# nh273/caro-ai

Hardware: AMD Instinct MI355X
Metric: self-play MCTS node-expansions/sec/GPU (Connect4, 200 sims/move); 1->8 GPU scaling (higher is better)
Workload: dtype f32

## Files before the change

caro_ai_amd/csrc/caro_engine.hip:

```cpp
#include <hip/hip_runtime.h>

#include <cstddef>
#include <cstdio>
#include <cstdlib>
#include <cstring>
#include <string>
#include <type_traits>
#include <vector>

#include "../../include/caro_hip.h"
#include "../../include/caro_noise.h"
#include "caro_rules.h"
#include "caro_variants.h"

namespace caro {

constexpr uint32_t NSTRONG = 1u << 30;
constexpr uint32_t NMASK = NSTRONG - 1u;
constexpr int ST_DROPPED = 0, ST_TERMINAL = 1, ST_LEAF = 2;
constexpr int MAXB = 64;
constexpr int DONE_HELD = 3;

enum Counter { C_SIMS, C_LEVELS, C_EXPANSIONS, C_TERMINALS, C_DROPPED, C_OVERFLOW, C_PLIES, C_FINISHED, C_N };

// ... 1099 lines not shown
    float* dst = planes + (size_t)rowi * 2 * HW;
    for (int i = tid; i < 2 * HW; i += blockDim.x) dst[i] = R::plane(v.gp, brd, who, i / HW, i % HW);
    if (leaf_keys && tid < KW) leaf_keys[(size_t)rowi * KW + tid] = v.d_key[di * KW + tid];
  }
}

template <int AP>
__device__ __forceinline__ void backup_path(const View& v, int t, float value, bool strong_val, const int32_t* pn,
                                            const int32_t* pa, int len) {
  float cur = -value;
  for (int i = len - 1; i >= 0; --i) {
    uint32_t* row = v.edges + (ebase(v, t) + pn[i]) * 4 * AP;
    const int a = pa[i];
    const uint32_t nraw = row[4 * a];
    const int n = (int)(nraw & NMASK) + 1;
    const uint32_t strong = (nraw & NSTRONG) | (strong_val ? NSTRONG : 0u);
    const float w = __uint_as_float(row[4 * a + 1]) + cur;
    const float q = w / (float)n;
    row[4 * a] = (uint32_t)n | strong;
    row[4 * a + 1] = __float_as_uint(w);
    row[4 * a + 2] = __float_as_uint(q);
    cur = -cur;
  }
}
template <int AP>
__device__ __forceinline__ void backup_path_rec(const View& v, int t, float value, bool strong_val, const uint4* rec,
                                                int len) {
  float cur = -value;
  for (int i = len - 1; i >= 0; --i) {
    const uint32_t na = rec[i].x;
    uint32_t* row = v.edges + (ebase(v, t) + (na & 0xFFFFFFu)) * 4 * AP;
    const int a = (int)(na >> 24);
    const uint32_t nraw = row[4 * a];
    const int n = (int)(nraw & NMASK) + 1;
    const uint32_t strong = (nraw & NSTRONG) | (strong_val ? NSTRONG : 0u);
    const float w = __uint_as_float(row[4 * a + 1]) + cur;
    row[4 * a] = (uint32_t)n | strong;
    row[4 * a + 1] = __float_as_uint(w);
    row[4 * a + 2] = __float_as_uint(w / (float)n);
    cur = -cur;
  }
}

template <class GEO>
struct ExpandPre {
  static constexpr int NPR = (MAXB * 0 + 64 * GEO::APL + 63) / 64;
  uint4 rec;
  typename GEO::R::Board brd;
  float row_val;
  uint4 p0, p1;
  float pr[NPR];
  int nleaf;
};
template <class GEO, bool ONE>
__device__ __forceinline__ ExpandPre<GEO> expand_preload(const View& v, int g, int B, int off, const float* __restrict__ probs,
                                                         const float* __restrict__ values) {
  using R = typename GEO::R;
  constexpr int KW = GEO::KW, AP = GEO::AP;
  ExpandPre<GEO> e;
  const int lane = threadIdx.x;
  e.nleaf = v.g_nleaf[g];
  e.rec = make_uint4(ST_DROPPED, 0u, 0u, 0u);
  e.row_val = 0.f;
#pragma unroll
  for (int w = 0; w < KW; ++w) e.brd.w[w] = 0;
  if (lane < B) {
    const size_t di = (size_t)g * v.maxB + lane;
    e.rec = v.d_rec[di];
    e.brd = load_board<R>(v.d_key + di * KW);
    if ((long long)off + lane < (long long)v.G * v.maxB) e.row_val = values[off + lane];
  }
  e.p0 = e.p1 = make_uint4(0u, 0u, 0u, 0u);
  if (B <= 8 && lane < 64 && (lane >> 3) < B) {
    const uint4* pr = v.path_rec + ((size_t)g * v.maxB + (lane >> 3)) * v.maxd;
    if ((lane & 7) < v.maxd) e.p0 = pr[lane & 7];
    if (8 + (lane & 7) < v.maxd) e.p1 = pr[8 + (lane & 7)];
  }
#pragma unroll
  for (int k = 0; k < ExpandPre<GEO>::NPR; ++k) {
    e.pr[k] = 0.f;
    if (ONE) {
      const int idx = lane + 64 * k, b = idx / AP, a = idx - b * AP;
      if (idx < B * AP && a < v.A && lane < 64) e.pr[k] = probs[(size_t)(off + b) * v.A + a];
    }
  }
  return e;
}

template <class GEO, bool ONE = false, class OPT = TreeFull>
__device__ __forceinline__ void expand_body(const View& v, GameRegs<GEO>& gr, int B, const ExpandPre<GEO>& pre, int off,
                                            const float* __restrict__ probs) {
  using R = typename GEO::R;
  using Board = typename R::Board;
  constexpr int AP = GEO::AP, KW = GEO::KW;
  constexpr int MAXE = GEO::APL > 1 ? 256 : 512;
  constexpr int MAXB = geo_max_batch<GEO>();
  __shared__ int e_node[MAXE];
  __shared__ short e_act[MAXE];
  __shared__ float e_val[MAXE];
  __shared__ unsigned char e_strong[MAXE];
  __shared__ uint32_t e_n[MAXE], e_w[MAXE];
  __shared__ int s_total;
  __shared__ uint64_t s_brd[MAXB][KW];
  __shared__ int s_node[MAXB], s_row[MAXB];
  __shared__ uint32_t s_home[MAXB];
  __shared__ unsigned char s_free[MAXB];
  __shared__ int q_len[MAXB], q_off[MAXB], q_b[MAXB];
  __shared__ float q_val[MAXB];
  __shared__ unsigned char q_strong[MAXB];
  __shared__ int s_nq;
  __shared__ uint4 s_p0[64], s_p1[64];
  __shared__ float s_rowval[MAXB];
  const int g = blockIdx.x;
  if (gr.done) return;
  const int lane = threadIdx.x;
  unsigned long long* xs = dbg<OPT>(v) ? dbg<OPT>(v) + ((size_t)v.G + g) * 8 : nullptr;
#define CARO_XS(n) if (xs && lane == 0) xs[n] = __builtin_amdgcn_s_memtime();
  CARO_XS(0)
  const int st_sel = n_stores<OPT>(v) == 2 ? gr.player : 0;
  const int t = g * n_stores<OPT>(v) + st_sel;
  const int nleaf = pre.nleaf;
  const int base = st_sel ? gr.nn[1] : gr.nn[0];
  const bool overflow = base + nleaf > v.cap;
  const int A = v.A;
  const int tsel = st_sel ? gr.tbl[1] : gr.tbl[0];
  const size_t tb = tbase_sel(v, t, tsel);
  const size_t eb = ebase_sel(v, t, tsel);
  const int my_st = (int)(pre.rec.x & 0xFFu), my_len = (int)((pre.rec.x >> 8) & 0xFFu);
  const int my_local = (int)((pre.rec.x >> 16) & 0xFFu);
  const uint32_t my_home = pre.rec.z;
  float my_val = __uint_as_float(pre.rec.y);
  const Board& brd = pre.brd;
  const bool pre_paths = B <= 8 && block_threads<ONE>() >= 64;
  if (pre_paths && lane < 64) {
    s_p0[lane] = pre.p0;
    s_p1[lane] = pre.p1;
  }
  const bool is_leaf = lane < B && my_st == ST_LEAF && !overflow;
  if (lane < B) s_rowval[lane] = pre.row_val;
  block_sync<ONE>();
  if (lane < B) {
    s_node[lane] = -2;
    if (is_leaf) {
      my_val = s_rowval[my_local];
      s_home[lane] = my_home & 0x7fffffffu;
      s_free[lane] = (my_home >> 31) != 0u;
      s_row[lane] = off + my_local;
      s_node[lane] = -1;
#pragma unroll
      for (int w = 0; w < KW; ++w) s_brd[lane][w] = brd.w[w];
    }
  }
  block_sync<ONE>();
  CARO_XS(1)
  const bool whole_wave = ONE || blockDim.x >= 64;
  const bool wave0 = whole_wave && lane < 64;
  if (!overflow) {
    if (wave0) {
      bool clash = false;
      for (int bb = 0; bb < B; ++bb) {
        const int ob = __builtin_amdgcn_readlane((int)is_leaf, bb);
        const uint32_t oh = (uint32_t)__builtin_amdgcn_readlane((int)(my_home & 0x7fffffffu), bb);
        clash = clash || (bb < lane && ob && oh == (my_home & 0x7fffffffu));
      }
      const bool fast = is_leaf && (my_home >> 31) != 0u && !clash;
      if (fast) {
        uint64_t* k = v.node_key + (tb + (my_home & 0x7fffffffu)) * KW;
#pragma unroll
        for (int w = KW - 1; w >= 0; --w) k[w] = brd.w[w];
        s_node[lane] = (int)(my_home & 0x7fffffffu);
      }
      const unsigned long long slow = __ballot(is_leaf && !fast);
      if (slow) {
        asm volatile("" ::: "memory");
        __builtin_amdgcn_wave_barrier();
        if (lane == 0)
          for (unsigned long long m = slow; m; m &= m - 1ull) {
            const int b = __ffsll(m) - 1;
            Board lb;
#pragma unroll
            for (int w = 0; w < KW; ++w) lb.w[w] = s_brd[b][w];
            s_node[b] = insert_key<R>(v, t, lb);
          }
      }
    } else if (!whole_wave && lane == 0) {
      for (int b = 0; b < B; ++b) {
        if (s_node[b] == -2) continue;
        Board lb;
#pragma unroll
        for (int w = 0; w < KW; ++w) lb.w[w] = s_brd[b][w];
        s_node[b] = insert_key<R>(v, t, lb);
      }
    }
    if (lane == 0) {
      unsigned long long* ctr = v.counters + (size_t)g * C_N;
      v.n_nodes[t] = base + nleaf;
      atomicAdd(v.n_created + t, nleaf);
      atomicAdd(ctr + C_EXPANSIONS, (unsigned long long)nleaf);
    }
    if (st_sel) gr.nn[1] = base + nleaf;
    else gr.nn[0] = base + nleaf;
  } else if (lane == 0) {
    atomicAdd(v.counters + (size_t)g * C_N + C_OVERFLOW, 1ull);
  }
  CARO_XS(2)
  const unsigned long long m_term = __ballot(lane < B && my_st == ST_TERMINAL);
  const unsigned long long m_leaf = __ballot(is_leaf);
  const int n_term = __popcll(m_term);
  const unsigned long long below = (1ull << lane) - 1ull;
  int qpos = -1;
  if (lane < B && my_st == ST_TERMINAL) qpos = __popcll(m_term & below);
  else if (is_leaf) qpos = n_term + __popcll(m_leaf & below);
  if (qpos >= 0) {
    q_len[qpos] = my_len;
    q_b[qpos] = lane;
    q_val[qpos] = my_val;
    q_strong[qpos] = my_st == ST_LEAF;
  }
  if (lane == 0) s_nq = n_term + __popcll(m_leaf);
  block_sync<ONE>();
  const int nq = s_nq;
  if (lane == 0) {
    int acc = 0;
    for (int k = 0; k < nq; ++k) {
      q_off[k] = acc;
      acc += q_len[k];
    }
    s_total = acc;
  }
  block_sync<ONE>();
  CARO_XS(3)
  const int total = s_total;
  if (total <= MAXE)
    for (int j = lane; j < total; j += block_threads<ONE>()) {
      int k = 0;
      while (k + 1 < nq && q_off[k + 1] <= j) ++k;
      const int r = j - q_off[k];
      const int i = q_len[k] - 1 - r;
      uint4 rec;
      if (pre_paths && i < 8) rec = s_p0[q_b[k] * 8 + i];
      else if (pre_paths && i < 16) rec = s_p1[q_b[k] * 8 + i - 8];
      else rec = v.path_rec[((size_t)g * v.maxB + q_b[k]) * v.maxd + i];
      e_node[j] = (int)(rec.x & 0xFFFFFFu);
      e_act[j] = (short)(rec.x >> 24);
      e_n[j] = rec.y;
      e_w[j] = rec.z;
      e_val[j] = (r & 1) ? q_val[k] : -q_val[k];
      e_strong[j] = q_strong[k];
    }
  CARO_XS(4)
  if (!overflow)
    for (int idx = lane; idx < B * AP; idx += block_threads<ONE>()) {
      const int b = idx / AP, a = idx - b * AP;
      const int node = s_node[b];
      float pv = 0.f;
      if (ONE) {
        const int src = node >= 0 ? (s_row[b] - off) * AP + a : lane;
#pragma unroll
        for (int k = 0; k < ExpandPre<GEO>::NPR; ++k) {
          const float x = __shfl(pre.pr[k], src & 63, 64);
          pv = (src >> 6) == k ? x : pv;
        }
      } else if (node >= 0 && a < A) {
        pv = probs[(size_t)s_row[b] * A + a];
      }
      if (node < 0) continue;
      uint32_t* row = v.edges + (eb + node) * 4 * AP;
      if (a >= A) pv = 0.f;
      reinterpret_cast<uint4*>(row)[a] = make_uint4(0u, 0u, 0u, __float_as_uint(pv));
    }
  if (total > MAXE) {
    if (lane == 0)
      for (int k = 0; k < nq; ++k) {
        const size_t di = (size_t)g * v.maxB + q_b[k];
        backup_path_rec<AP>(v, t, q_val[k], q_strong[k] != 0, v.path_rec + di * v.maxd, q_len[k]);
      }
    return;
  }
  block_sync<ONE>();
  CARO_XS(5)
  const int n = total;
  if (whole_wave && n <= 128) {
    if (wave0) {
    const int j0 = lane, j1 = lane + 64;
    const bool v0 = j0 < n, v1 = j1 < n;
    const int key0 = v0 ? (e_node[j0] << 8) | (int)(unsigned short)e_act[j0] : -1;
    const int key1 = v1 ? (e_node[j1] << 8) | (int)(unsigned short)e_act[j1] : -1;
    unsigned long long todo0 = __ballot(v0), todo1 = __ballot(v1);
    bool own0 = false, own1 = false;
    unsigned long long g0m0 = 0ull, g0m1 = 0ull, g1m1 = 0ull;
    while (todo0 | todo1) {
      const bool lo = todo0 != 0ull;
      const int lead = lo ? __ffsll((unsigned long long)todo0) - 1 : __ffsll((unsigned long long)todo1) - 1;
      const int k = lo ? __builtin_amdgcn_readlane(key0, lead) : __builtin_amdgcn_readlane(key1, lead);
      const unsigned long long m0 = __ballot(v0 && key0 == k);
      const unsigned long long m1 = __ballot(v1 && key1 == k);
      if (lane == lead) {
        if (lo) { own0 = true; g0m0 = m0; g0m1 = m1; }
        else { own1 = true; g1m1 = m1; }
      }
      todo0 &= ~m0;
      todo1 &= ~m1;
    }
    uint32_t* row0 = own0 ? v.edges + (eb + (key0 >> 8)) * 4 * AP : nullptr;
    uint32_t* row1 = own1 ? v.edges + (eb + (key1 >> 8)) * 4 * AP : nullptr;
    const int a0 = key0 & 0xff, a1 = key1 & 0xff;
    if (own0) {
      const uint32_t n0 = e_n[j0];
      int cnt = (int)(n0 & NMASK);
      uint32_t strong = n0 & NSTRONG;
      float w = __uint_as_float(e_w[j0]);
      for (unsigned long long m = g0m0; m; m &= m - 1ull) {
        const int e = __ffsll(m) - 1;
        cnt += 1;
        w = w + e_val[e];
        if (e_strong[e]) strong = NSTRONG;
      }
      for (unsigned long long m = g0m1; m; m &= m - 1ull) {
        const int e = 64 + __ffsll(m) - 1;
        cnt += 1;
        w = w + e_val[e];
        if (e_strong[e]) strong = NSTRONG;
      }
// ... 22 lines not shown
    const int node = e_node[j], a = e_act[j];
    bool owner = true;
    for (int k = 0; k < j; ++k) owner = owner && !(e_node[k] == node && e_act[k] == a);
    if (!owner) continue;
    uint32_t* row = v.edges + (eb + node) * 4 * AP;
    const uint32_t nraw = e_n[j];
    int cnt = (int)(nraw & NMASK);
    uint32_t strong = nraw & NSTRONG;
    float w = __uint_as_float(e_w[j]);
    for (int k = j; k < n; ++k) {
      if (e_node[k] == node && e_act[k] == a) {
        cnt += 1;
        w = w + e_val[k];
        if (e_strong[k]) strong = NSTRONG;
      }
    }
    row[4 * a] = (uint32_t)cnt | strong;
    row[4 * a + 1] = __float_as_uint(w);
    row[4 * a + 2] = __float_as_uint(w / (float)cnt);
  }
  CARO_XS(6)
  if (xs && lane == 0) xs[7] = (unsigned long long)total;
#undef CARO_XS
}

template <class GEO>
__global__ void k_expand_backup(View v, const float* __restrict__ probs, const float* __restrict__ values) {
  GameRegs<GEO> gr = load_game<GEO>(v, blockIdx.x);
  const int B = v.leaf_count[2], off = v.g_off[blockIdx.x];
  const ExpandPre<GEO> pre = expand_preload<GEO, false>(v, blockIdx.x, B, off, probs, values);
  expand_body<GEO>(v, gr, B, pre, off, probs);
}

template <class GEO>
__device__ __forceinline__ void noise_wave(const View& v, int B, int go, uint64_t uid, uint32_t ply, int mb,
                                           double* s_nz, volatile int* s_flag) {
  constexpr int LPD = GEO::LPD, APL = GEO::APL, AP = GEO::AP;
  const int lane = threadIdx.x & 63;
  const int b = lane / LPD, l = lane % LPD;
  if (go) {
    double nz[APL];
    const uint64_t key = caro_noise_key(v.seed, uid, ply, (uint32_t)(mb * B + b));
    __shared__ double s_mail[APL > 1 ? 2 * AP : 1];
    noise_group<LPD, APL>(key, l, v.A, v.alpha, nz, s_mail);
#pragma unroll
    for (int j = 0; j < APL; ++j) s_nz[b * AP + l * APL + j] = nz[j];
  }
  __builtin_amdgcn_fence(__ATOMIC_RELEASE, "workgroup");
  __builtin_amdgcn_wave_barrier();
  if (lane == 0) *s_flag = 1;
}

template <class GEO, class OPT>
__global__ void k_tree(View v, int B, int mb_index, const double* __restrict__ noise, const float* __restrict__ probs,
                       const float* __restrict__ values, float* __restrict__ planes, uint64_t* __restrict__ leaf_keys,
                       int32_t* __restrict__ rows_cur, int32_t* __restrict__ rows_next, int do_expand,
                       int do_select) {
  __shared__ double s_nz[MAXB * 0 + 64 * GEO::APL];
  __shared__ int s_flag;
  if (threadIdx.x == 0) s_flag = 0;
  __syncthreads();
  if (threadIdx.x >= 64) {
    const int g = blockIdx.x;
    const int go = do_select && !noise && !v.done[g] && !(cap_on<OPT>(v) && mb_index >= v.cap_fast && v.fast[g]) &&
                   !(es_on<OPT>(v) && mb_index > 0 && v.es_cut[g]);
    noise_wave<GEO>(v, B, go, go ? v.uid[g] : 0ull, go ? (uint32_t)v.ply[g] : 0u, mb_index, s_nz, &s_flag);
    return;
  }
  __builtin_amdgcn_s_setprio(3);
  if (blockIdx.x == 0 && threadIdx.x == 0) {
    rows_next[0] = 0;
    rows_next[1] = 0;
    rows_next[2] = B;
    rows_cur[2] = B;
  }
  unsigned long long t0 = 0;
  if (dbg<OPT>(v)) t0 = __builtin_amdgcn_s_memtime();
  GameRegs<GEO> gr = load_game<GEO, OPT>(v, blockIdx.x);
  const ExpandPre<GEO> pre = expand_preload<GEO, true>(v, blockIdx.x, B, blockIdx.x * B, probs, values);
  if (do_expand) {
    expand_body<GEO, true, OPT>(v, gr, B, pre, blockIdx.x * B, probs);
    block_sync<true>();
  }
  const unsigned long long t1 = dbg<OPT>(v) ? __builtin_amdgcn_s_memtime() : 0;
  if (dbg<OPT>(v) && threadIdx.x == 0 && !do_select) dbg<OPT>(v)[(size_t)blockIdx.x * 8 + 5] = t1 - t0;
  if (do_select) select_body<GEO, true, OPT>(v, gr, B, mb_index, noise, rows_cur, planes, leaf_keys, s_nz, &s_flag);
  if (dbg<OPT>(v) && threadIdx.x == 0 && do_select) {
    dbg<OPT>(v)[(size_t)blockIdx.x * 8 + 6] = t1 - t0;
    dbg<OPT>(v)[(size_t)blockIdx.x * 8 + 7] = __builtin_amdgcn_s_memtime() - t0;
  }
}

template <bool ONE>
__device__ __forceinline__ void lds_temperature(int A, int AP, double tau, int best, int nmax, double total,
                                                const int* s_n, double* s_pi, double* s_sum) {
  const bool general = tau != 0.0 && tau != 1.0;
  for (int a = threadIdx.x; a < AP; a += block_threads<ONE>()) {
    double p = 0.0;
    if (a < A) {
      if (tau == 0.0) p = a == best ? 1.0 : 0.0;
      else if (!general) p = (double)s_n[a] / total;
      else p = temp_weight(s_n[a], nmax, tau);
    }
    s_pi[a] = p;
  }
  block_sync<ONE>();
  if (general) {
    if (threadIdx.x == 0) {
      double S = 0.0;
      for (int a = 0; a < A; ++a) S = S + s_pi[a];
      *s_sum = S;
    }
    block_sync<ONE>();
    const double S = *s_sum;
    for (int a = threadIdx.x; a < A; a += block_threads<ONE>()) s_pi[a] = s_pi[a] / S;
    block_sync<ONE>();
  }
}

template <class GEO>
__device__ __forceinline__ void root_policy(const View& v, int g, int t, const typename GEO::R::Board& root,
                                            double* s_pi, int* s_n) {
  using R = typename GEO::R;
  constexpr int AP = GEO::AP;
  const int node = probe<R>(v, t, root);
  for (int a = threadIdx.x; a < AP; a += blockDim.x)
    s_n[a] = (node >= 0 && a < v.A) ? (int)(v.edges[((ebase(v, t) + node) * AP + a) * 4] & NMASK) : 0;
  __syncthreads();
  __shared__ int s_best;
  __shared__ double s_total, s_sum;
  if (threadIdx.x == 0) {
    int best = 0;
    long long tot = 0;
    for (int a = 0; a < v.A; ++a) {
      if (s_n[a] > s_n[best]) best = a;
      tot += s_n[a];
// ... 546 lines not shown
    const Opened<GEO> o = opening_of<GEO>(v.gp, v.seed, nuid, fp, v.open_n);
    gr.root = o.root;
    fp = o.player;
    made = o.made;
  }
  gr.player = fp;
  gr.ply = 0;
  gr.step = 0;
  gr.uid = nuid;
  gr.done = 0;
  const bool flip = v.etab != 2;
#pragma unroll
  for (int st = 0; st < 2; ++st) {
    if (flip) gr.tbl[st] = 1 - gr.tbl[st];
    gr.nn[st] = 0;
  }
  if (threadIdx.x == 0) {
#pragma unroll
    for (int st = 0; st < 2; ++st) {
      if (st < n_stores<OPT>(v)) {
        const int t = g * n_stores<OPT>(v) + st;
        if (flip) {
          v.tbl[t] = gr.tbl[st];
          v.dirty[t] = 1;
        }
        v.n_nodes[t] = 0;
        v.n_created[t] = 0;
      }
    }
    store_board<R>(v.root + (size_t)g * KW, gr.root);
    v.player[g] = fp;
    v.first[g] = fp;
    v.ply[g] = 0;
    v.step[g] = 0;
    v.uid[g] = nuid;
    v.done[g] = 0;
    v.result[g] = 0;
    v.final_r[g] = 0;
    if (open_made<OPT>(v)) open_made<OPT>(v)[g] = (int16_t)made;
    if (cap_on<OPT>(v)) v.fast[g] = cap_is_fast(v, nuid, 0);
    if (es_on<OPT>(v)) es_ply_start(v, g);
  }
  return true;
}

template <class GEO, class OPT>
__global__ void k_tree_stag(View v, int B, const float* __restrict__ probs, const float* __restrict__ values,
                            float* __restrict__ planes, uint64_t* __restrict__ leaf_keys,
                            int32_t* __restrict__ rows_cur, int32_t* __restrict__ rows_next) {
  constexpr int AP = GEO::AP;
  __shared__ double s_pi[AP];
  __shared__ int s_n[AP];
  __shared__ double s_nz[64 * GEO::APL];
  __shared__ int s_flag;
  const int g = blockIdx.x;
  if (threadIdx.x == 0) s_flag = 0;
  const int w = v.wait[g];
  int lm = v.lm[g];
  const int pend = v.pend[g];
  const int due = (cap_on<OPT>(v) && v.fast[g]) ? v.cap_fast : v.stag_S;
  const int cut = es_on<OPT>(v) ? v.es_cut[g] : 0;
  GameRegs<GEO> gr = load_game<GEO, OPT>(v, g);
  ExpandPre<GEO> pre;
  if (threadIdx.x < 64) pre = expand_preload<GEO, true>(v, g, B, g * B, probs, values);
  __syncthreads();
  if (threadIdx.x >= 64) {
    const int go = w == 0 && gr.done == 0;
    int lm_h = go ? lm : 0;
    uint32_t ply_h = go ? (uint32_t)gr.ply : 0u;
    if (lm_h >= due || (go && cut)) {
      lm_h = 0;
      ply_h += 1u;
    }
    noise_wave<GEO>(v, B, go, go ? gr.uid : 0ull, ply_h, lm_h, s_nz, &s_flag);
    return;
  }
  __builtin_amdgcn_s_setprio(3);
  if (blockIdx.x == 0 && threadIdx.x == 0) {
    rows_next[0] = 0;
    rows_next[1] = 0;
    rows_next[2] = B;
    rows_cur[2] = B;
  }
  const unsigned long long t0 = dbg<OPT>(v) ? __builtin_amdgcn_s_memtime() : 0;
  if (w > 0) {
    if (threadIdx.x == 0) {
      v.wait[g] = w - 1;
      v.g_nleaf[g] = 0;
      v.g_class[g] = 0;
      v.g_pack[g] = 0;
    }
    return;
  }
  if (gr.done == 2) {
    if (threadIdx.x == 0) {
      v.g_nleaf[g] = 0;
      v.g_class[g] = 0;
      v.g_pack[g] = 0;
    }
    return;
  }
  if (pend) {
    expand_body<GEO, true, OPT>(v, gr, B, pre, g * B, probs);
    block_sync<true>();
  }
  const unsigned long long t1 = dbg<OPT>(v) ? __builtin_amdgcn_s_memtime() : 0;
  int over = gr.done == 1;
  if (!over && (lm >= due || cut)) {
    over = step_body<GEO, true, OPT>(v, g, gr, nullptr, s_pi, s_n, nullptr, nullptr, nullptr);
    lm = 0;
  }
  if (over) {
    if (park_and_restart<GEO, true, OPT>(v, g, gr)) over = 0;
  }
  const unsigned long long t2 = dbg<OPT>(v) ? __builtin_amdgcn_s_memtime() : 0;
  select_body<GEO, true, OPT>(v, gr, B, lm, nullptr, rows_cur, planes, leaf_keys, s_nz, &s_flag);
  if (threadIdx.x == 0) {
    v.lm[g] = over ? 0 : lm + 1;
    v.pend[g] = over ? 0 : 1;
    if (dbg<OPT>(v)) {
      dbg<OPT>(v)[(size_t)g * 8 + 5] = ((t2 - t1) & 0xFFFFFFull) | (__builtin_amdgcn_s_memrealtime() << 24);
      dbg<OPT>(v)[(size_t)g * 8 + 6] = t1 - t0;
      dbg<OPT>(v)[(size_t)g * 8 + 7] = __builtin_amdgcn_s_memtime() - t0;
      dbg<OPT>(v)[(size_t)g * 8 + 4] |= (unsigned long long)__builtin_amdgcn_s_getreg((31 << 11) | 4) << 8;
    }
  }
}

template <class GEO, class OPT = TreeFull>
__global__ void k_tree_stag_mw(View v, int B, const float* __restrict__ probs, const float* __restrict__ values,
                               float* __restrict__ planes, uint64_t* __restrict__ leaf_keys,
                               int32_t* __restrict__ rows_cur, int32_t* __restrict__ rows_next) {
  constexpr int AP = GEO::AP;
  __shared__ double s_pi[AP];
  __shared__ int s_n[AP];
  const int g = blockIdx.x;
  if (g == 0 && threadIdx.x == 0) {
    rows_next[0] = 0;
    rows_next[1] = 0;
    rows_next[2] = B;
    rows_cur[2] = B;
  }
  const int w = v.wait[g];
  int lm = v.lm[g];
  const int pend = v.pend[g];
  const int due = (v.cap_on && v.fast[g]) ? v.cap_fast : v.stag_S;
  const int cut = v.es_on ? v.es_cut[g] : 0;
  GameRegs<GEO> gr = load_game<GEO>(v, g);
  const ExpandPre<GEO> pre = expand_preload<GEO, false>(v, g, B, g * B, probs, values);
  __syncthreads();
  if (w > 0 || gr.done == 2) {
    if (threadIdx.x == 0) {
      if (w > 0) v.wait[g] = w - 1;
      v.g_nleaf[g] = 0;
      v.g_class[g] = 0;
      v.g_pack[g] = 0;
    }
// ... 1421 lines not shown

int caro_leaf_counts(caro_engine* h, int32_t counts[2], void* stream) {
  if (!h || !counts) return fail(CARO_E_INVAL, "null argument");
  HIPCHK(hipMemcpyAsync(h->pinned, h->v.leaf_count, 2 * sizeof(int32_t), hipMemcpyDeviceToHost, (hipStream_t)stream));
  HIPCHK(hipStreamSynchronize((hipStream_t)stream));
  counts[0] = h->pinned[0];
  counts[1] = h->pinned[1];
  return 0;
}

int caro_expand_backup(caro_engine* h, const float* probs, const float* values, void* stream) {
  if (!h) return fail(CARO_E_INVAL, "null engine");
  if (!h->select_pending) return fail(CARO_E_STATE, "caro_expand_backup without a pending caro_select");
  const int p0 = prof_begin(h, PK_EXPAND, (hipStream_t)stream);
  DISPATCH(h->var, hipLaunchKernelGGL(k_expand_backup<GEO>, dim3(h->v.G), dim3(64), 0, (hipStream_t)stream, h->v,
                                      probs, values));
  prof_end(h, p0, (hipStream_t)stream);
  HIPCHK(hipGetLastError());
  h->select_pending = 0;
  return 0;
}

static int search_batch_impl(caro_engine* h, caro_net* net0, caro_net* net1, int searches, int batch, const double* noise,
                             float* planes, uint64_t* leaf_keys, float* probs, float* values, void* stream, int with_step,
                             const double* uniforms, int32_t* actions, int32_t* done, int32_t* result) {
  if (!h || !net0 || !planes || !probs || !values) return fail(CARO_E_INVAL, "null argument");
  if (h->v.n_nets == 2 && !net1) return fail(CARO_E_INVAL, "engine has two nets, net1 is null");
  if (searches < 1) return fail(CARO_E_INVAL, "searches must be >= 1");
  const int64_t max_rows = (int64_t)h->v.G * batch;
  const size_t noise_stride = (size_t)h->v.G * batch * h->v.A;
  if (batch < 1 || batch > h->v.maxB) return fail(CARO_E_INVAL, "batch exceeds max_batch of the engine");
  if (h->v.stag_S) return fail(CARO_E_STATE, "caro_search_batch: the engine runs in staggered mode (per-game clocks, pending minibatches, parked games); use caro_search_staggered / caro_drain_parked_begin");
  if (h->select_pending) return fail(CARO_E_STATE, "caro_search_batch with a pending caro_select");
  hipStream_t st = (hipStream_t)stream;
  const int bthreads = batch * variant_lpd(h->var);
  const bool fused1 = h->fused_ok && bthreads == 64;
  const bool fused = h->fused_ok && bthreads >= 64 && bthreads % 64 == 0;
  h->ls_mid = 1;
  View sv = h->v;
  sv.ls_M = searches;
  if (!caro_net_uses_slot_list(net0)) sv.slot_list = nullptr;
  for (int mb = 0; mb < searches; ++mb) {
    h->prof_gate = (h->prof_ctr++ % PROF_EVERY) == 0;
    int rc = 0;
    const int32_t* counts = h->v.leaf_count;
    if (fused) {
      int32_t* cur = h->rows + 4 * h->rows_par;
      int32_t* nxt = h->rows + 4 * (h->rows_par ^ 1);
      h->rows_par ^= 1;
      counts = cur;
      const int p1 = prof_begin(h, PK_SELECT, st);
      if (fused1) {
        if (tree_lean(h)) {
          DISPATCH(h->var, hipLaunchKernelGGL(HIP_KERNEL_NAME(k_tree<GEO, TreeLean>), dim3(h->v.G), dim3(128), 0, st, sv,
                                              batch, mb, noise ? noise + (size_t)mb * noise_stride : nullptr, probs,
                                              values, planes, leaf_keys, cur, nxt, mb > 0 ? 1 : 0, 1));
        } else if (tree_vl(h, batch)) {
          DISPATCH(h->var, hipLaunchKernelGGL(HIP_KERNEL_NAME(k_tree<GEO, TreeVl>), dim3(h->v.G), dim3(128), 0, st, sv,
                                              batch, mb, noise ? noise + (size_t)mb * noise_stride : nullptr, probs,
                                              values, planes, leaf_keys, cur, nxt, mb > 0 ? 1 : 0, 1));
        } else {
          DISPATCH(h->var, hipLaunchKernelGGL(HIP_KERNEL_NAME(k_tree<GEO, TreeFull>), dim3(h->v.G), dim3(128), 0, st, sv,
                                              batch, mb, noise ? noise + (size_t)mb * noise_stride : nullptr, probs,
                                              values, planes, leaf_keys, cur, nxt, mb > 0 ? 1 : 0, 1));
        }
      } else if (tree_vl(h, batch)) {
        DISPATCH(h->var, hipLaunchKernelGGL(HIP_KERNEL_NAME(k_tree_mw<GEO, TreeVl>), dim3(h->v.G), dim3(bthreads),
                                            mail_bytes<GEO>(batch), st, sv, batch, mb,
                                            noise ? noise + (size_t)mb * noise_stride : nullptr, probs, values, planes,
                                            leaf_keys, cur, nxt, mb > 0 ? 1 : 0, 1, 0, (const double*)nullptr,
                                            (int32_t*)nullptr, (int32_t*)nullptr, (int32_t*)nullptr));
      } else {
        DISPATCH(h->var, hipLaunchKernelGGL(k_tree_mw<GEO>, dim3(h->v.G), dim3(bthreads), mail_bytes<GEO>(batch), st,
                                            sv, batch, mb, noise ? noise + (size_t)mb * noise_stride : nullptr, probs,
                                            values, planes, leaf_keys, cur, nxt, mb > 0 ? 1 : 0, 1, 0,
                                            (const double*)nullptr, (int32_t*)nullptr, (int32_t*)nullptr,
                                            (int32_t*)nullptr));
      }
      prof_end(h, p1, st);
      if (hipGetLastError() != hipSuccess) { h->prof_gate = 1; return fail(CARO_E_HIP, "k_tree launch failed"); }
    } else {
      rc = select_impl(h, batch, mb, searches, noise ? noise + (size_t)mb * noise_stride : nullptr, planes, leaf_keys,
                       stream);
      if (rc) { h->prof_gate = 1; return rc; }
    }
    const int p0 = prof_begin(h, PK_NET, st);
    if (fused)
      rc = caro_net_forward_slot_list(net0, h->v.n_nets == 2 ? net1 : nullptr, planes, counts, h->v.g_pack,
                                      fused1 ? nullptr : sv.slot_list, h->v.G, batch, probs, values, stream);
    else if (h->v.n_nets == 2)
      rc = caro_net_forward_pair_at(net0, net1, planes, counts, -1, max_rows, probs, values, stream);
    else rc = caro_net_forward(net0, planes, counts, 0, max_rows, probs, values, stream);
    prof_end(h, p0, st);
    prof_calibrate(h, st);
    if (!rc && !fused) rc = caro_expand_backup(h, probs, values, stream);
    if (rc) { h->prof_gate = 1; return rc; }
  }
  if (fused) {
    int32_t* cur = h->rows + 4 * h->rows_par;
    int32_t* nxt = h->rows + 4 * (h->rows_par ^ 1);
    h->rows_par ^= 1;
    const int p1 = prof_begin(h, PK_EXPAND, st);
    if (fused1) {
      if (tree_lean(h)) {
        DISPATCH(h->var, hipLaunchKernelGGL(HIP_KERNEL_NAME(k_tree<GEO, TreeLean>), dim3(h->v.G), dim3(128), 0, st, h->v,
                                            batch, searches, (const double*)nullptr, probs, values, planes, leaf_keys,
                                            cur, nxt, 1, 0));
      } else {
        DISPATCH(h->var, hipLaunchKernelGGL(HIP_KERNEL_NAME(k_tree<GEO, TreeFull>), dim3(h->v.G), dim3(128), 0, st, h->v,
                                            batch, searches, (const double*)nullptr, probs, values, planes, leaf_keys,
                                            cur, nxt, 1, 0));
      }
    } else {
      DISPATCH(h->var, hipLaunchKernelGGL(k_tree_mw<GEO>, dim3(h->v.G), dim3(bthreads), 0, st, h->v, batch, searches,
                                          (const double*)nullptr, probs, values, planes, leaf_keys, cur, nxt, 1, 0,
                                          with_step ? 1 : 0, uniforms, actions, done, result));
      if (with_step) {
        with_step = 0;
        h->ls_mid = 0;
        h->ls_forced = 0;
      }
    }
    prof_end(h, p1, st);
    if (hipGetLastError() != hipSuccess) { h->prof_gate = 1; return fail(CARO_E_HIP, "k_tree launch failed"); }
  }
  h->prof_gate = 1;
  return with_step ? caro_step(h, uniforms, actions, done, result, stream) : 0;
}

int caro_search_batch(caro_engine* h, caro_net* net0, caro_net* net1, int searches, int batch, const double* noise,
                      float* planes, uint64_t* leaf_keys, float* probs, float* values, void* stream) {
  return search_batch_impl(h, net0, net1, searches, batch, noise, planes, leaf_keys, probs, values, stream, 0, nullptr,
                           nullptr, nullptr, nullptr);
}

int caro_search_move(caro_engine* h, caro_net* net0, caro_net* net1, int searches, int batch, const double* noise,
                     const double* uniforms, float* planes, uint64_t* leaf_keys, float* probs, float* values,
                     int32_t* actions, int32_t* done, int32_t* result, void* stream) {
  return search_batch_impl(h, net0, net1, searches, batch, noise, planes, leaf_keys, probs, values, stream, 1, uniforms,
                           actions, done, result);
}

int caro_search_staggered(caro_engine* h, caro_net* net0, caro_net* net1, int launches, int batch, float* planes,
                          uint64_t* leaf_keys, float* probs, float* values, void* stream) {
  if (!h || !net0 || !planes || !probs || !values) return fail(CARO_E_INVAL, "null argument");
  if (!h->v.stag_S) return fail(CARO_E_STATE, "the engine was not created in staggered mode (caro_config.stagger)");
  if (h->v.n_nets == 2 && !net1) return fail(CARO_E_INVAL, "engine has two nets, net1 is null");
  if (launches < 1) return fail(CARO_E_INVAL, "launches must be >= 1");
  const int bthreads = batch * variant_lpd(h->var);
  if (batch < 1 || batch > h->v.maxB || bthreads < 64 || bthreads % 64 != 0)
    return fail(CARO_E_INVAL, "staggered mode: batch x lanes per descent must be a multiple of 64");
  if (h->cfg.evict && bthreads == 64)
    return fail(CARO_E_INVAL, "staggered mode with eviction: batch x lanes per descent must be above 64");
  if (h->stag_batch && h->stag_batch != batch) return fail(CARO_E_INVAL, "staggered mode: the batch size is fixed by the first call");
  h->stag_batch = batch;
  hipStream_t st = (hipStream_t)stream;
  View sv = h->v;
  if (!caro_net_uses_slot_list(net0)) sv.slot_list = nullptr;
  for (int j = 0; j < launches; ++j) {
    h->prof_gate = (h->prof_ctr++ % PROF_EVERY) == 0;
    int32_t* cur = h->rows + 4 * h->rows_par;
    int32_t* nxt = h->rows + 4 * (h->rows_par ^ 1);
    h->rows_par ^= 1;
    const int p1 = prof_begin(h, PK_SELECT, st);
    if (bthreads == 64 && tree_lean(h)) {
      DISPATCH(h->var, hipLaunchKernelGGL(HIP_KERNEL_NAME(k_tree_stag<GEO, TreeLean>), dim3(h->v.G), dim3(128), 0, st,
                                          h->v, batch, probs, values, planes, leaf_keys, cur, nxt));
    } else if (bthreads == 64 && tree_vl(h, batch)) {
      DISPATCH(h->var, hipLaunchKernelGGL(HIP_KERNEL_NAME(k_tree_stag<GEO, TreeVl>), dim3(h->v.G), dim3(128), 0, st,
                                          h->v, batch, probs, values, planes, leaf_keys, cur, nxt));
    } else if (bthreads == 64) {
      DISPATCH(h->var, hipLaunchKernelGGL(HIP_KERNEL_NAME(k_tree_stag<GEO, TreeFull>), dim3(h->v.G), dim3(128), 0, st,
                                          h->v, batch, probs, values, planes, leaf_keys, cur, nxt));
    } else if (tree_vl(h, batch)) {
      DISPATCH(h->var, hipLaunchKernelGGL(HIP_KERNEL_NAME(k_tree_stag_mw<GEO, TreeVl>), dim3(h->v.G), dim3(bthreads),
                                          mail_bytes<GEO>(batch), st, sv, batch, probs, values, planes, leaf_keys, cur,
                                          nxt));
    } else {
      DISPATCH(h->var, hipLaunchKernelGGL(k_tree_stag_mw<GEO>, dim3(h->v.G), dim3(bthreads), mail_bytes<GEO>(batch), st,
                                          sv, batch, probs, values, planes, leaf_keys, cur, nxt));
    }
    prof_end(h, p1, st);
    if (hipGetLastError() != hipSuccess) { h->prof_gate = 1; return fail(CARO_E_HIP, "k_tree_stag launch failed"); }
    const int p0 = prof_begin(h, PK_NET, st);
    const int rc = caro_net_forward_slot_list(net0, h->v.n_nets == 2 ? net1 : nullptr, planes, cur, h->v.g_pack,
                                              bthreads == 64 ? nullptr : sv.slot_list, h->v.G, batch, probs, values,
                                              stream);
    prof_end(h, p0, st);
    prof_calibrate(h, st);
    if (rc) { h->prof_gate = 1; return rc; }
    if (h->v.stag_pool && j % 5 == 4)
      DISPATCH(h->var, hipLaunchKernelGGL(k_stag_assign<GEO>, dim3(1), dim3(1024), 0, st, h->v));
  }
  h->prof_gate = 1;
  return 0;
}

int caro_drain_parked_begin(caro_engine* h, int64_t cap, uint64_t* states, int32_t* players, double* pi, int32_t* z,
                            int64_t* games, void* stream) {
  return caro_drain_parked_begin_q(h, cap, states, players, pi, z, games, nullptr, stream);
}
int caro_drain_parked_begin_q(caro_engine* h, int64_t cap, uint64_t* states, int32_t* players, double* pi, int32_t* z,
                              int64_t* games, double* root_q, void* stream) {
  return caro_drain_parked_begin_x(h, cap, states, players, pi, z, games, root_q, nullptr, stream);
}
int caro_drain_parked_begin_x(caro_engine* h, int64_t cap, uint64_t* states, int32_t* players, double* pi, int32_t* z,
                              int64_t* games, double* root_q, uint8_t* full, void* stream) {
  caro_drain_extra ex = {(uint32_t)sizeof(caro_drain_extra), root_q, full, nullptr, nullptr};
  return caro_drain_parked_begin_ex(h, cap, states, players, pi, z, games, &ex, stream);
}
static int drain_extra(const caro_drain_extra* in, caro_drain_extra* out) {
  *out = caro_drain_extra{(uint32_t)sizeof(caro_drain_extra), nullptr, nullptr, nullptr, nullptr};
  if (!in) return 0;
  if (in->size < offsetof(caro_drain_extra, root_q_dev)) return fail(CARO_E_INVAL, "caro_drain_extra.size is not set");
  if (in->size >= offsetof(caro_drain_extra, root_q_dev) + sizeof(double*)) out->root_q_dev = in->root_q_dev;
  if (in->size >= offsetof(caro_drain_extra, full_dev) + sizeof(uint8_t*)) out->full_dev = in->full_dev;
  if (in->size >= offsetof(caro_drain_extra, minibatches_dev) + sizeof(uint16_t*)) out->minibatches_dev = in->minibatches_dev;
  if (in->size >= offsetof(caro_drain_extra, open_dev) + sizeof(int16_t*)) out->open_dev = in->open_dev;
  return 0;
}
int caro_drain_parked_begin_ex(caro_engine* h, int64_t cap, uint64_t* states, int32_t* players, double* pi, int32_t* z,
                               int64_t* games, const caro_drain_extra* extra, void* stream) {
  if (!h || !states || !players || !pi || !z) return fail(CARO_E_INVAL, "null argument");
  caro_drain_extra ex;
  if (int rc = drain_extra(extra, &ex)) return rc;
// ... 337 lines not shown
```

Baseline: 8.510 million.

## Split expansion into a dedicated node-insertion wave running alongside backup

Adds a third wavefront to the fused one-wave tree kernels. It performs hash-table node insertion and edge-row writes, while wave 0 does only the value backup. A shared-memory flag with release/acquire fences makes wave 0 wait for the node wave before selection. The aim is to overlap the serial insert_key work with backup and preloading. In exchange, each block uses more threads and extra registers, and the spin-wait adds synchronisation overhead.

After: 8.562 million, median of 6. No clear change (+0.6%).

```diff
diff --git a/caro_ai_amd/csrc/caro_engine.hip b/caro_ai_amd/csrc/caro_engine.hip
--- a/caro_ai_amd/csrc/caro_engine.hip
+++ b/caro_ai_amd/csrc/caro_engine.hip
@@ -1175,13 +1175,15 @@
   float pr[NPR];
   int nleaf;
 };
-template <class GEO, bool ONE>
+enum { EX_ALL = 0, EX_BACKUP = 1, EX_NODES = 2 };
+template <class GEO, bool ONE, int ROLE = EX_ALL>
 __device__ __forceinline__ ExpandPre<GEO> expand_preload(const View& v, int g, int B, int off, const float* __restrict__ probs,
                                                          const float* __restrict__ values) {
   using R = typename GEO::R;
   constexpr int KW = GEO::KW, AP = GEO::AP;
+  static_assert(ROLE == EX_ALL || ONE, "the split forms are the one-wave kernels'");
   ExpandPre<GEO> e;
-  const int lane = threadIdx.x;
+  const int lane = ROLE == EX_NODES ? (int)(threadIdx.x & 63) : (int)threadIdx.x;
   e.nleaf = v.g_nleaf[g];
   e.rec = make_uint4(ST_DROPPED, 0u, 0u, 0u);
   e.row_val = 0.f;
@@ -1190,11 +1192,12 @@
   if (lane < B) {
     const size_t di = (size_t)g * v.maxB + lane;
     e.rec = v.d_rec[di];
-    e.brd = load_board<R>(v.d_key + di * KW);
-    if ((long long)off + lane < (long long)v.G * v.maxB) e.row_val = values[off + lane];
+    if (ROLE != EX_BACKUP) e.brd = load_board<R>(v.d_key + di * KW);
+    if (ROLE != EX_NODES)
+      if ((long long)off + lane < (long long)v.G * v.maxB) e.row_val = values[off + lane];
   }
   e.p0 = e.p1 = make_uint4(0u, 0u, 0u, 0u);
-  if (B <= 8 && lane < 64 && (lane >> 3) < B) {
+  if (ROLE != EX_NODES && B <= 8 && lane < 64 && (lane >> 3) < B) {
     const uint4* pr = v.path_rec + ((size_t)g * v.maxB + (lane >> 3)) * v.maxd;
     if ((lane & 7) < v.maxd) e.p0 = pr[lane & 7];
     if (8 + (lane & 7) < v.maxd) e.p1 = pr[8 + (lane & 7)];
@@ -1202,7 +1205,7 @@
 #pragma unroll
   for (int k = 0; k < ExpandPre<GEO>::NPR; ++k) {
     e.pr[k] = 0.f;
-    if (ONE) {
+    if (ONE && ROLE != EX_BACKUP) {
       const int idx = lane + 64 * k, b = idx / AP, a = idx - b * AP;
       if (idx < B * AP && a < v.A && lane < 64) e.pr[k] = probs[(size_t)(off + b) * v.A + a];
     }
@@ -1210,7 +1213,7 @@
   return e;
 }
 
-template <class GEO, bool ONE = false, class OPT = TreeFull>
+template <class GEO, bool ONE = false, class OPT = TreeFull, int ROLE = EX_ALL>
 __device__ __forceinline__ void expand_body(const View& v, GameRegs<GEO>& gr, int B, const ExpandPre<GEO>& pre, int off,
                                             const float* __restrict__ probs) {
   using R = typename GEO::R;
@@ -1234,10 +1237,11 @@
   __shared__ int s_nq;
   __shared__ uint4 s_p0[64], s_p1[64];
   __shared__ float s_rowval[MAXB];
+  static_assert(ROLE == EX_ALL || ONE, "the split forms are the one-wave kernels'");
   const int g = blockIdx.x;
   if (gr.done) return;
-  const int lane = threadIdx.x;
-  unsigned long long* xs = dbg<OPT>(v) ? dbg<OPT>(v) + ((size_t)v.G + g) * 8 : nullptr;
+  const int lane = ROLE == EX_NODES ? (int)(threadIdx.x & 63) : (int)threadIdx.x;
+  unsigned long long* xs = dbg<OPT>(v) && ROLE != EX_NODES ? dbg<OPT>(v) + ((size_t)v.G + g) * 8 : nullptr;
 #define CARO_XS(n) if (xs && lane == 0) xs[n] = __builtin_amdgcn_s_memtime();
   CARO_XS(0)
   const int st_sel = n_stores<OPT>(v) == 2 ? gr.player : 0;
@@ -1255,17 +1259,20 @@
   float my_val = __uint_as_float(pre.rec.y);
   const Board& brd = pre.brd;
   const bool pre_paths = B <= 8 && block_threads<ONE>() >= 64;
-  if (pre_paths && lane < 64) {
+  if (ROLE == EX_NODES && overflow) return;
+  if (ROLE != EX_NODES && pre_paths && lane < 64) {
     s_p0[lane] = pre.p0;
     s_p1[lane] = pre.p1;
   }
   const bool is_leaf = lane < B && my_st == ST_LEAF && !overflow;
-  if (lane < B) s_rowval[lane] = pre.row_val;
+  if (ROLE != EX_NODES && lane < B) s_rowval[lane] = pre.row_val;
   block_sync<ONE>();
-  if (lane < B) {
+  if (ROLE == EX_BACKUP) {
+    if (is_leaf) my_val = s_rowval[my_local];
+  } else if (lane < B) {
     s_node[lane] = -2;
     if (is_leaf) {
-      my_val = s_rowval[my_local];
+      if (ROLE != EX_NODES) my_val = s_rowval[my_local];
       s_home[lane] = my_home & 0x7fffffffu;
       s_free[lane] = (my_home >> 31) != 0u;
       s_row[lane] = off + my_local;
@@ -1279,7 +1286,8 @@
   const bool whole_wave = ONE || blockDim.x >= 64;
   const bool wave0 = whole_wave && lane < 64;
   if (!overflow) {
-    if (wave0) {
+    if (ROLE == EX_BACKUP) {
+    } else if (wave0) {
       bool clash = false;
       for (int bb = 0; bb < B; ++bb) {
         const int ob = __builtin_amdgcn_readlane((int)is_leaf, bb);
@@ -1315,7 +1323,7 @@
         s_node[b] = insert_key<R>(v, t, lb);
       }
     }
-    if (lane == 0) {
+    if (ROLE != EX_BACKUP && lane == 0) {
       unsigned long long* ctr = v.counters + (size_t)g * C_N;
       v.n_nodes[t] = base + nleaf;
       atomicAdd(v.n_created + t, nleaf);
@@ -1326,7 +1334,33 @@
   } else if (lane == 0) {
     atomicAdd(v.counters + (size_t)g * C_N + C_OVERFLOW, 1ull);
   }
+  const auto write_rows = [&]() {
+    for (int idx = lane; idx < B * AP; idx += block_threads<ONE>()) {
+      const int b = idx / AP, a = idx - b * AP;
+      const int node = s_node[b];
+      float pv = 0.f;
+      if (ONE) {
+        const int src = node >= 0 ? (s_row[b] - off) * AP + a : lane;
+#pragma unroll
+        for (int k = 0; k < ExpandPre<GEO>::NPR; ++k) {
+          const float x = __shfl(pre.pr[k], src & 63, 64);
+          pv = (src >> 6) == k ? x : pv;
+        }
+      } else if (node >= 0 && a < A) {
+        pv = probs[(size_t)s_row[b] * A + a];
+      }
+      if (node < 0) continue;
+      uint32_t* row = v.edges + (eb + node) * 4 * AP;
+      if (a >= A) pv = 0.f;
+      reinterpret_cast<uint4*>(row)[a] = make_uint4(0u, 0u, 0u, __float_as_uint(pv));
+    }
+  };
   CARO_XS(2)
+  if constexpr (ROLE == EX_NODES) {
+    block_sync<ONE>();
+    write_rows();
+    return;
+  }
   const unsigned long long m_term = __ballot(lane < B && my_st == ST_TERMINAL);
   const unsigned long long m_leaf = __ballot(is_leaf);
   const int n_term = __popcll(m_term);
@@ -1372,26 +1406,7 @@
       e_strong[j] = q_strong[k];
     }
   CARO_XS(4)
-  if (!overflow)
-    for (int idx = lane; idx < B * AP; idx += block_threads<ONE>()) {
-      const int b = idx / AP, a = idx - b * AP;
-      const int node = s_node[b];
-      float pv = 0.f;
-      if (ONE) {
-        const int src = node >= 0 ? (s_row[b] - off) * AP + a : lane;
-#pragma unroll
-        for (int k = 0; k < ExpandPre<GEO>::NPR; ++k) {
-          const float x = __shfl(pre.pr[k], src & 63, 64);
-          pv = (src >> 6) == k ? x : pv;
-        }
-      } else if (node >= 0 && a < A) {
-        pv = probs[(size_t)s_row[b] * A + a];
-      }
-      if (node < 0) continue;
-      uint32_t* row = v.edges + (eb + node) * 4 * AP;
-      if (a >= A) pv = 0.f;
-      reinterpret_cast<uint4*>(row)[a] = make_uint4(0u, 0u, 0u, __float_as_uint(pv));
-    }
+  if (ROLE == EX_ALL && !overflow) write_rows();
   if (total > MAXE) {
     if (lane == 0)
       for (int k = 0; k < nq; ++k) {
@@ -1520,14 +1535,44 @@
 }
 
 template <class GEO, class OPT>
+__device__ __forceinline__ void node_wave(const View& v, GameRegs<GEO>& gr, int B, int go, const ExpandPre<GEO>& pre,
+                                          int off, const float* __restrict__ probs, volatile int* s_flag) {
+  __builtin_amdgcn_s_setprio(2);
+  if (go) expand_body<GEO, true, OPT, EX_NODES>(v, gr, B, pre, off, probs);
+  asm volatile("s_waitcnt vmcnt(0)" ::: "memory");
+  __builtin_amdgcn_fence(__ATOMIC_RELEASE, "workgroup");
+  __builtin_amdgcn_wave_barrier();
+  if ((threadIdx.x & 63) == 0) *s_flag = 1;
+}
+__device__ __forceinline__ void node_wave_wait(volatile int* s_flag) {
+  while (*s_flag == 0) __builtin_amdgcn_s_sleep(1);
+  __builtin_amdgcn_fence(__ATOMIC_ACQUIRE, "workgroup");
+}
+
+template <class GEO, class OPT>
 __global__ void k_tree(View v, int B, int mb_index, const double* __restrict__ noise, const float* __restrict__ probs,
                        const float* __restrict__ values, float* __restrict__ planes, uint64_t* __restrict__ leaf_keys,
                        int32_t* __restrict__ rows_cur, int32_t* __restrict__ rows_next, int do_expand,
                        int do_select) {
   __shared__ double s_nz[MAXB * 0 + 64 * GEO::APL];
-  __shared__ int s_flag;
-  if (threadIdx.x == 0) s_flag = 0;
+  __shared__ int s_flag, s_nflag;
+  if (threadIdx.x == 0) s_flag = s_nflag = 0;
+  unsigned long long t0 = 0;
+  if (dbg<OPT>(v)) t0 = __builtin_amdgcn_s_memtime();
+  GameRegs<GEO> gr;
+  ExpandPre<GEO> pre;
+  if (threadIdx.x < 64) {
+    gr = load_game<GEO, OPT>(v, blockIdx.x);
+    pre = expand_preload<GEO, true, EX_BACKUP>(v, blockIdx.x, B, blockIdx.x * B, probs, values);
+  } else if (threadIdx.x >= 128) {
+    gr = load_game<GEO, OPT>(v, blockIdx.x);
+    pre = expand_preload<GEO, true, EX_NODES>(v, blockIdx.x, B, blockIdx.x * B, probs, values);
+  }
   __syncthreads();
+  if (threadIdx.x >= 128) {
+    node_wave<GEO, OPT>(v, gr, B, do_expand, pre, blockIdx.x * B, probs, &s_nflag);
+    return;
+  }
   if (threadIdx.x >= 64) {
     const int g = blockIdx.x;
     const int go = do_select && !noise && !v.done[g] && !(cap_on<OPT>(v) && mb_index >= v.cap_fast && v.fast[g]) &&
@@ -1542,14 +1587,11 @@
     rows_next[2] = B;
     rows_cur[2] = B;
   }
-  unsigned long long t0 = 0;
-  if (dbg<OPT>(v)) t0 = __builtin_amdgcn_s_memtime();
-  GameRegs<GEO> gr = load_game<GEO, OPT>(v, blockIdx.x);
-  const ExpandPre<GEO> pre = expand_preload<GEO, true>(v, blockIdx.x, B, blockIdx.x * B, probs, values);
   if (do_expand) {
-    expand_body<GEO, true, OPT>(v, gr, B, pre, blockIdx.x * B, probs);
+    expand_body<GEO, true, OPT, EX_BACKUP>(v, gr, B, pre, blockIdx.x * B, probs);
     block_sync<true>();
   }
+  node_wave_wait(&s_nflag);
   const unsigned long long t1 = dbg<OPT>(v) ? __builtin_amdgcn_s_memtime() : 0;
   if (dbg<OPT>(v) && threadIdx.x == 0 && !do_select) dbg<OPT>(v)[(size_t)blockIdx.x * 8 + 5] = t1 - t0;
   if (do_select) select_body<GEO, true, OPT>(v, gr, B, mb_index, noise, rows_cur, planes, leaf_keys, s_nz, &s_flag);
@@ -2202,9 +2244,9 @@
   __shared__ double s_pi[AP];
   __shared__ int s_n[AP];
   __shared__ double s_nz[64 * GEO::APL];
-  __shared__ int s_flag;
+  __shared__ int s_flag, s_nflag;
   const int g = blockIdx.x;
-  if (threadIdx.x == 0) s_flag = 0;
+  if (threadIdx.x == 0) s_flag = s_nflag = 0;
   const int w = v.wait[g];
   int lm = v.lm[g];
   const int pend = v.pend[g];
@@ -2212,8 +2254,13 @@
   const int cut = es_on<OPT>(v) ? v.es_cut[g] : 0;
   GameRegs<GEO> gr = load_game<GEO, OPT>(v, g);
   ExpandPre<GEO> pre;
-  if (threadIdx.x < 64) pre = expand_preload<GEO, true>(v, g, B, g * B, probs, values);
+  if (threadIdx.x < 64) pre = expand_preload<GEO, true, EX_BACKUP>(v, g, B, g * B, probs, values);
+  else if (threadIdx.x >= 128) pre = expand_preload<GEO, true, EX_NODES>(v, g, B, g * B, probs, values);
   __syncthreads();
+  if (threadIdx.x >= 128) {
+    node_wave<GEO, OPT>(v, gr, B, w == 0 && gr.done != 2 && pend, pre, g * B, probs, &s_nflag);
+    return;
+  }
   if (threadIdx.x >= 64) {
     const int go = w == 0 && gr.done == 0;
     int lm_h = go ? lm : 0;
@@ -2251,8 +2298,9 @@
     return;
   }
   if (pend) {
-    expand_body<GEO, true, OPT>(v, gr, B, pre, g * B, probs);
+    expand_body<GEO, true, OPT, EX_BACKUP>(v, gr, B, pre, g * B, probs);
     block_sync<true>();
+    node_wave_wait(&s_nflag);
   }
   const unsigned long long t1 = dbg<OPT>(v) ? __builtin_amdgcn_s_memtime() : 0;
   int over = gr.done == 1;
@@ -3780,15 +3828,15 @@
       const int p1 = prof_begin(h, PK_SELECT, st);
       if (fused1) {
         if (tree_lean(h)) {
-          DISPATCH(h->var, hipLaunchKernelGGL(HIP_KERNEL_NAME(k_tree<GEO, TreeLean>), dim3(h->v.G), dim3(128), 0, st, sv,
+          DISPATCH(h->var, hipLaunchKernelGGL(HIP_KERNEL_NAME(k_tree<GEO, TreeLean>), dim3(h->v.G), dim3(192), 0, st, sv,
                                               batch, mb, noise ? noise + (size_t)mb * noise_stride : nullptr, probs,
                                               values, planes, leaf_keys, cur, nxt, mb > 0 ? 1 : 0, 1));
         } else if (tree_vl(h, batch)) {
-          DISPATCH(h->var, hipLaunchKernelGGL(HIP_KERNEL_NAME(k_tree<GEO, TreeVl>), dim3(h->v.G), dim3(128), 0, st, sv,
+          DISPATCH(h->var, hipLaunchKernelGGL(HIP_KERNEL_NAME(k_tree<GEO, TreeVl>), dim3(h->v.G), dim3(192), 0, st, sv,
                                               batch, mb, noise ? noise + (size_t)mb * noise_stride : nullptr, probs,
                                               values, planes, leaf_keys, cur, nxt, mb > 0 ? 1 : 0, 1));
         } else {
-          DISPATCH(h->var, hipLaunchKernelGGL(HIP_KERNEL_NAME(k_tree<GEO, TreeFull>), dim3(h->v.G), dim3(128), 0, st, sv,
+          DISPATCH(h->var, hipLaunchKernelGGL(HIP_KERNEL_NAME(k_tree<GEO, TreeFull>), dim3(h->v.G), dim3(192), 0, st, sv,
                                               batch, mb, noise ? noise + (size_t)mb * noise_stride : nullptr, probs,
                                               values, planes, leaf_keys, cur, nxt, mb > 0 ? 1 : 0, 1));
         }
@@ -3831,11 +3879,11 @@
     const int p1 = prof_begin(h, PK_EXPAND, st);
     if (fused1) {
       if (tree_lean(h)) {
-        DISPATCH(h->var, hipLaunchKernelGGL(HIP_KERNEL_NAME(k_tree<GEO, TreeLean>), dim3(h->v.G), dim3(128), 0, st, h->v,
+        DISPATCH(h->var, hipLaunchKernelGGL(HIP_KERNEL_NAME(k_tree<GEO, TreeLean>), dim3(h->v.G), dim3(192), 0, st, h->v,
                                             batch, searches, (const double*)nullptr, probs, values, planes, leaf_keys,
                                             cur, nxt, 1, 0));
       } else {
-        DISPATCH(h->var, hipLaunchKernelGGL(HIP_KERNEL_NAME(k_tree<GEO, TreeFull>), dim3(h->v.G), dim3(128), 0, st, h->v,
+        DISPATCH(h->var, hipLaunchKernelGGL(HIP_KERNEL_NAME(k_tree<GEO, TreeFull>), dim3(h->v.G), dim3(192), 0, st, h->v,
                                             batch, searches, (const double*)nullptr, probs, values, planes, leaf_keys,
                                             cur, nxt, 1, 0));
       }
@@ -3892,13 +3940,13 @@
     h->rows_par ^= 1;
     const int p1 = prof_begin(h, PK_SELECT, st);
     if (bthreads == 64 && tree_lean(h)) {
-      DISPATCH(h->var, hipLaunchKernelGGL(HIP_KERNEL_NAME(k_tree_stag<GEO, TreeLean>), dim3(h->v.G), dim3(128), 0, st,
+      DISPATCH(h->var, hipLaunchKernelGGL(HIP_KERNEL_NAME(k_tree_stag<GEO, TreeLean>), dim3(h->v.G), dim3(192), 0, st,
                                           h->v, batch, probs, values, planes, leaf_keys, cur, nxt));
     } else if (bthreads == 64 && tree_vl(h, batch)) {
-      DISPATCH(h->var, hipLaunchKernelGGL(HIP_KERNEL_NAME(k_tree_stag<GEO, TreeVl>), dim3(h->v.G), dim3(128), 0, st,
+      DISPATCH(h->var, hipLaunchKernelGGL(HIP_KERNEL_NAME(k_tree_stag<GEO, TreeVl>), dim3(h->v.G), dim3(192), 0, st,
                                           h->v, batch, probs, values, planes, leaf_keys, cur, nxt));
     } else if (bthreads == 64) {
-      DISPATCH(h->var, hipLaunchKernelGGL(HIP_KERNEL_NAME(k_tree_stag<GEO, TreeFull>), dim3(h->v.G), dim3(128), 0, st,
+      DISPATCH(h->var, hipLaunchKernelGGL(HIP_KERNEL_NAME(k_tree_stag<GEO, TreeFull>), dim3(h->v.G), dim3(192), 0, st,
                                           h->v, batch, probs, values, planes, leaf_keys, cur, nxt));
     } else if (tree_vl(h, batch)) {
       DISPATCH(h->var, hipLaunchKernelGGL(HIP_KERNEL_NAME(k_tree_stag_mw<GEO, TreeVl>), dim3(h->v.G), dim3(bthreads),
```
